# toastori/zig-flac

Hardware: AMD Instinct MI355X
Metric: MSamples/s encoded (whole node), 44.1kHz/16-bit stereo, blocksize 4096 (higher is better)
Workload: dtype int32

## Files before the change

### zig-flac_amd/csrc/fg_crc.hpp

```cpp
#pragma once
#include <stdint.h>

#ifndef FG_HD
#if defined(__HIPCC__)
#define FG_HD __host__ __device__ __forceinline__
#else
#define FG_HD inline
#endif
#endif

namespace fg {

FG_HD uint32_t q_fold(uint32_t t) {
    const uint32_t h = t >> 15;
    return (t & 0x7FFFu) ^ h ^ (h << 1);
}
FG_HD uint32_t q_word(uint32_t s, uint32_t W) { return q_fold(W ^ (s << 4) ^ (s << 2)); }
FG_HD uint32_t q_mul(uint32_t a, uint32_t e) {
    uint32_t r = 0;
#pragma unroll
    for (int i = 0; i < 15; i++) r ^= (e << i) & (uint32_t)(-(int32_t)((a >> i) & 1u));
    return q_fold(r);
}
FG_HD uint32_t crc_from_q(uint32_t qp) {
    const uint32_t A = qp & 0x7FFFu;
    return A ^ (((__builtin_popcount(A) ^ (qp >> 16)) & 1u) ? 0x8003u : 0u);
}
FG_HD uint32_t crc_lane_q(const uint32_t *img, int32_t va, uint32_t n, uint32_t e) {
    uint32_t s = 0, px = 0;
    for (uint32_t i = va < 0 ? (uint32_t)(-va) : 0u; i < n; i++) {
        const uint32_t w = img[va + (int32_t)i];
        s = q_word(s, w);
        px ^= w;
    }
    return q_mul(q_fold(s), e) | ((__builtin_popcount(px) & 1u) << 16);
}
FG_HD uint32_t crc_byte_v(uint32_t crc, uint32_t b) {
    const uint32_t t = ((crc >> 8) ^ b) & 255u;
    return ((crc << 8) ^ (t << 1) ^ (t << 2) ^ ((__builtin_popcount(t) & 1u) ? 0x8003u : 0u)) & 0xFFFFu;
}
FG_HD uint32_t crc_mulmod_v(uint32_t a, uint32_t b) {
    uint32_t t[16];
#pragma unroll
    for (int i = 0; i < 16; i++) t[i] = (b << i) & (uint32_t)(-(int32_t)((a >> i) & 1u));
#pragma unroll
    for (int w = 8; w >= 1; w >>= 1)
#pragma unroll
        for (int i = 0; i < w; i++) t[i] ^= t[i + w];
    return crc_from_q(q_fold(q_fold(t[0])) | ((__builtin_popcount(t[0]) & 1u) << 16));
}

}
```

### zig-flac_amd/csrc/fg_device.hpp

```cpp
#pragma once
#include <hip/hip_runtime.h>
#include <cstdlib>
#include <mutex>
#include <type_traits>

#include "fg_common.hpp"
#include "fg_crc.hpp"
#include "fg_layout.hpp"

namespace fg {

template <uint32_t V>
using ic = std::integral_constant<uint32_t, V>;
template <typename T>
struct tyt {
    using type = T;
};

__device__ __forceinline__ uint32_t lane_id() { return __lane_id(); }
__device__ __forceinline__ uint32_t opaque(uint32_t v) {
    asm volatile("" : "+v"(v));
    return v;
}

__device__ __forceinline__ uint32_t sad_u32(uint32_t a, uint32_t b, uint32_t acc) {
    uint32_t d;
    asm("v_sad_u32 %0, %1, %2, %3" : "=v"(d) : "v"(a), "v"(b), "v"(acc));
    return d;
}

__device__ __forceinline__ uint32_t add_chain(uint32_t a, uint32_t b) {
    uint32_t d;
    asm("v_add_u32 %0, %1, %2" : "=v"(d) : "v"(a), "v"(b));
    return d;
}

enum : int {
    DPP_XOR1 = 0xB1,
    DPP_XOR2 = 0x4E,
    DPP_SHR1 = 0x111,
    DPP_SHR2 = 0x112,
    DPP_SHR4 = 0x114,
    DPP_SHR8 = 0x118,
    DPP_WSHR1 = 0x138,
    DPP_MIRROR = 0x140,
    DPP_HMIRROR = 0x141,
    DPP_BCAST15 = 0x142,
    DPP_BCAST31 = 0x143,
};

template <int CTRL, int RM = 0xF, int BM = 0xF, bool BC = true>
__device__ __forceinline__ uint32_t dpp(uint32_t v) {
    return (uint32_t)__builtin_amdgcn_update_dpp(0, (int)v, CTRL, RM, BM, BC);
}
template <int CTRL>
__device__ __forceinline__ uint64_t dpp64(uint64_t v) {
    return (uint64_t)dpp<CTRL>((uint32_t)v) | ((uint64_t)dpp<CTRL>((uint32_t)(v >> 32)) << 32);
}
__device__ __forceinline__ uint32_t rdl(uint32_t v, int lane) {
    return (uint32_t)__builtin_amdgcn_readlane((int)v, lane);
}
__device__ __forceinline__ uint64_t rdl64(uint64_t v, int lane) {
    return (uint64_t)rdl((uint32_t)v, lane) | ((uint64_t)rdl((uint32_t)(v >> 32), lane) << 32);
}

template <typename T>
__device__ __forceinline__ T dppT(T v, int which);
#define FG_ROW_REDUCE(NAME, T, OP, DPPF)                       \
    __device__ __forceinline__ T NAME(T v) {                   \
        v = OP(v, DPPF<DPP_XOR1>(v));                          \
        v = OP(v, DPPF<DPP_XOR2>(v));                          \
        v = OP(v, DPPF<DPP_HMIRROR>(v));                       \
        v = OP(v, DPPF<DPP_MIRROR>(v));                        \
        return v;                                              \
    }
#define FG_ADD(a, b) ((a) + (b))
#define FG_OR(a, b) ((a) | (b))
#define FG_XOR(a, b) ((a) ^ (b))
#ifndef FG_MAX
#define FG_MAX(a, b) max((a), (b))
#endif
#ifndef FG_LKEEP24
#define FG_LKEEP24 1
#endif
FG_ROW_REDUCE(row_sum32, uint32_t, FG_ADD, dpp)
FG_ROW_REDUCE(row_sum64, uint64_t, FG_ADD, dpp64)
FG_ROW_REDUCE(row_or32, uint32_t, FG_OR, dpp)
FG_ROW_REDUCE(row_or64, uint64_t, FG_OR, dpp64)
FG_ROW_REDUCE(row_xor32, uint32_t, FG_XOR, dpp)
FG_ROW_REDUCE(row_max32, uint32_t, FG_MAX, dpp)

__device__ __forceinline__ uint32_t wave_sum32(uint32_t v) {
    v = row_sum32(v);
    return rdl(v, 0) + rdl(v, 16) + rdl(v, 32) + rdl(v, 48);
}
__device__ __forceinline__ uint64_t wave_sum64(uint64_t v) {
    v = row_sum64(v);
    return rdl64(v, 0) + rdl64(v, 16) + rdl64(v, 32) + rdl64(v, 48);
}
__device__ __forceinline__ uint32_t wave_or32(uint32_t v) {
    v = row_or32(v);
    return rdl(v, 0) | rdl(v, 16) | rdl(v, 32) | rdl(v, 48);
}
__device__ __forceinline__ uint64_t wave_or64(uint64_t v) {
    v = row_or64(v);
    return rdl64(v, 0) | rdl64(v, 16) | rdl64(v, 32) | rdl64(v, 48);
}
__device__ __forceinline__ uint32_t wave_max32(uint32_t v) {
    v = row_max32(v);
    return max(max(rdl(v, 0), rdl(v, 16)), max(rdl(v, 32), rdl(v, 48)));
}
__device__ __forceinline__ uint32_t wave_xor32(uint32_t v) {
    v = row_xor32(v);
    return rdl(v, 0) ^ rdl(v, 16) ^ rdl(v, 32) ^ rdl(v, 48);
}
__device__ __forceinline__ uint32_t wave_incl_scan32(uint32_t x) {
    x += dpp<DPP_SHR1>(x);
    x += dpp<DPP_SHR2>(x);
    x += dpp<DPP_SHR4>(x);
    x += dpp<DPP_SHR8>(x);
    x += dpp<DPP_BCAST15, 0xA, 0xF, false>(x);
    x += dpp<DPP_BCAST31, 0xC, 0xF, false>(x);
    return x;
}
__device__ __forceinline__ uint32_t shr1_32(uint32_t v) { return dpp<DPP_WSHR1>(v); }
__device__ __forceinline__ int32_t shr1(int32_t v) { return (int32_t)shr1_32((uint32_t)v); }
__device__ __forceinline__ int64_t shr1(int64_t v) { return (int64_t)dpp64<DPP_WSHR1>((uint64_t)v); }

__device__ __forceinline__ uint32_t bitlen32(uint32_t x) { return x ? 32u - (uint32_t)__builtin_clz(x) : 0u; }
__device__ __forceinline__ uint32_t bitlen64(uint64_t x) { return x ? 64u - (uint32_t)__builtin_clzll(x) : 0u; }
__device__ __forceinline__ uint32_t zigzag32(int32_t r) { return ((uint32_t)r << 1) ^ (uint32_t)(r >> 31); }

__device__ __forceinline__ uint32_t rice_choose(uint64_t S, uint32_t len, uint32_t width, uint32_t maxp,
                                                uint32_t *cost) {
    uint32_t p;
    if (S <= (uint64_t)((len + 1u) >> 1)) {
        p = 0;
    } else {
        const uint64_t two = 2ull * len;
        uint32_t m = 0;
        if (S > two) {
            m = bitlen64(S) - bitlen64(two);
            if ((S >> m) > two) m++;
        }
        p = m + 1u;
    }
    if (p > maxp - 1u) p = maxp - 1u;
    const uint64_t f = (p == 0) ? (uint64_t)len + (S << 1)
                                : (uint64_t)(1u + p) * len + ((S >> (p - 1u)) - (uint64_t)(len >> 1));
    const uint64_t esc = (width <= 31u) ? 5ull + (uint64_t)width * len : ~0ull;
    if (f < esc) {
        *cost = (uint32_t)f;
        return p;
    }
    *cost = (uint32_t)esc;
    return 0x80u | width;
}

__device__ __forceinline__ uint32_t rice_choose(uint32_t S, uint32_t len, uint32_t width, uint32_t maxp,
                                                uint32_t *cost) {
    uint32_t p;
    if (S <= ((len + 1u) >> 1)) {
        p = 0;
    } else {
        const uint32_t two = 2u * len;
        uint32_t m = 0;
        if (S > two) {
            m = bitlen32(S) - bitlen32(two);
            if ((S >> m) > two) m++;
        }
        p = m + 1u;
    }
    if (p > maxp - 1u) p = maxp - 1u;
    const uint32_t f = (p == 0) ? len + (S << 1) : (1u + p) * len + ((S >> (p - 1u)) - (len >> 1));
    const uint32_t esc = (width <= 31u) ? 5u + width * len : ~0u;
    if (f < esc) {
        *cost = f;
        return p;
    }
    *cost = esc;
    return 0x80u | width;
}


__device__ __forceinline__ void lds_or2(uint32_t addr, uint32_t hi, uint32_t lo) {
    asm volatile("ds_or_b32 %0, %1\n\tds_or_b32 %0, %2 offset:4" ::"v"(addr), "v"(hi), "v"(lo) : "memory");
}

__device__ __forceinline__ void store_frame16(const uint32_t *img, uint8_t *out, uint64_t D, uint32_t fbytes,
                                              uint32_t tid, uint32_t NT, uint32_t lo = 0) {
    const uint64_t E = D + fbytes;
    const uint32_t sa = (uint32_t)(D & 3u);
    const uint64_t qD = D >> 2;
    const uint64_t DL = D + lo;
    const uint32_t r = (uint32_t)(qD & 3u);
    for (uint64_t u = (DL >> 4) + tid; u < ((E + 15u) >> 4); u += NT) {
        const int32_t m0 = (int32_t)(4u * u - qD);
        const int32_t a1 = m0 + (int32_t)r;
        const uint4 q1 = *(const uint4 *)(img + a1);
        const uint4 q0 = a1 >= 4 ? *(const uint4 *)(img + a1 - 4) : make_uint4(0, 0, 0, 0);
        const uint32_t w8[8] = {q0.x, q0.y, q0.z, q0.w, q1.x, q1.y, q1.z, q1.w};
        uint32_t wv[5];
#pragma unroll
        for (int c = 0; c < 5; c++)
            wv[c] = r == 0 ? w8[3 + c] : r == 1 ? w8[2 + c] : r == 2 ? w8[1 + c] : w8[c];
        uint32_t v[4];
        uint32_t prev = m0 >= 1 ? wv[0] : 0u;
#pragma unroll
        for (int c = 0; c < 4; c++) {
            const uint32_t lo = m0 + c >= 0 ? wv[c + 1] : 0u;
            v[c] = __builtin_bswap32(sa ? __builtin_amdgcn_alignbyte(prev, lo, sa) : lo);
            prev = lo;
        }
        const uint64_t b0 = 16u * u;
        if (b0 >= DL && b0 + 16u <= E) {
            *(uint4 *)(out + b0) = make_uint4(v[0], v[1], v[2], v[3]);
        } else {
#pragma unroll
            for (int c = 0; c < 4; c++)
#pragma unroll
                for (uint32_t b = 0; b < 4; b++) {
                    const uint64_t bb = b0 + 4u * c + b;
                    if (bb >= DL && bb < E) out[bb] = (uint8_t)(v[c] >> (8 * b));
                }
        }
    }
}

__device__ __forceinline__ void put_bits(uint32_t *img, uint32_t pos, uint64_t v, uint32_t len) {
    if (len == 0) return;
    const uint32_t wi = pos >> 5, o = pos & 31u;
    const uint64_t t = v << (64u - o - len);
    atomicOr(&img[wi], (uint32_t)(t >> 32));
    if (o + len > 32u) atomicOr(&img[wi + 1], (uint32_t)t);
}

__device__ __forceinline__ void put_or2(uint32_t *img, uint32_t pos, uint64_t v, uint32_t len) {
    const uint32_t wi = pos >> 5, o = pos & 31u;
    const uint64_t t = len ? (v << (64u - o - len)) : 0ull;
    atomicOr(&img[wi], (uint32_t)(t >> 32));
    atomicOr(&img[wi + 1], (uint32_t)t);
}

struct AtomicWriter {
    uint32_t *img;
    uint32_t pos;
    __device__ __forceinline__ void init(uint32_t *im, uint32_t bitpos) {
        img = im;
        pos = bitpos;
    }
    __device__ __forceinline__ void put(uint64_t v, uint32_t len) {
        put_bits(img, pos, v, len);
        pos += len;
    }
    __device__ __forceinline__ void zeros(uint32_t q) { pos += q; }
    __device__ __forceinline__ void finish() {}
};

struct HdrWriter {
    uint64_t accu = 0;
    uint64_t w0 = 0;
    uint32_t remain = 64;
    uint32_t end = 0;
    __device__ void bits(uint32_t n, uint64_t v) {
        if (n == 0) return;
        if (n <= remain) {
            accu = (n == 64) ? 0 : (accu << n);
            accu |= v;
            remain -= n;
        } else {
            const uint32_t sh = n - remain;
            accu = (remain == 64) ? 0 : (accu << remain);
            accu |= v >> sh;
            w0 = accu;
            end++;
            accu = v;
            remain = 64 - sh;
        }
    }
};

__device__ __forceinline__ uint32_t crc8_byte(uint32_t c, uint32_t b) {
    c ^= b;
#pragma unroll
    for (int i = 0; i < 8; i++) c = (c & 0x80u) ? ((c << 1) ^ 0x07u) & 0xFFu : (c << 1) & 0xFFu;
    return c;
}

__device__ __noinline__ uint32_t write_frame_header(uint32_t *img, uint64_t frame_number, uint32_t bits,
                                                    uint32_t channel_code, uint32_t block_size,
                                                    uint32_t sample_rate) {
    HdrWriter h;
    h.bits(16, 0xFFF8);
    uint32_t unc_bs = 0;
    const uint32_t ctz = (uint32_t)__builtin_ctz(block_size);
    if ((block_size & (block_size - 1u)) == 0 && ctz <= 15 && ctz >= 8) {
        h.bits(4, ctz);
    } else if (block_size == 192) {
        h.bits(4, 1);
    } else if ((block_size >> ctz) == 144 && ctz <= 5 && ctz >= 2) {
        h.bits(4, ctz);
    } else if (block_size < 0x100) {
        h.bits(4, 6);
        unc_bs = 8;
    } else {
        h.bits(4, 7);
        unc_bs = 16;
    }
    uint32_t unc_sr = 0, rc;
    switch (sample_rate) {
        case 0: rc = 0; break;
        case 88200: rc = 1; break;
        case 176400: rc = 2; break;
        case 192000: rc = 3; break;
        case 8000: rc = 4; break;
        case 16000: rc = 5; break;
        case 22050: rc = 6; break;
        case 24000: rc = 7; break;
        case 32000: rc = 8; break;
        case 44100: rc = 9; break;
        case 48000: rc = 10; break;
        case 96000: rc = 11; break;
        default:
            if (sample_rate <= 255) { unc_sr = 4; rc = 12; }
            else if (sample_rate <= 65535) { unc_sr = 1; rc = 13; }
            else { unc_sr = 10; rc = 14; }
    }
    h.bits(4, rc);
    h.bits(4, channel_code);
    h.bits(4, bits == 8 ? 2u : bits == 16 ? 8u : bits == 24 ? 12u : 14u);
    if (frame_number <= 0x7F) {
        h.bits(8, frame_number);
    } else {
        uint64_t buf = 0, num = frame_number, fbm = 0x3F;
        uint32_t i = 0;
        while (num > fbm) {
            buf |= (0x80ull + (num & 0x3F)) << (8 * i);
            i++;
            num >>= 6;
            fbm >>= 1;
        }
        buf |= ((0xFEull << (6 - i)) | num) << (8 * i);
        const uint32_t nb = 8 * (i + 1);
        h.bits(nb, buf & (~0ull >> (64 - nb)));
    }
    if (unc_bs) h.bits(unc_bs, block_size - 1u);
    if (unc_sr == 4) h.bits(8, block_size);
    else if (unc_sr) h.bits(16, block_size / unc_sr);
    const uint32_t byte_end = 8u - h.remain / 8u;
    const uint64_t a_al = (h.remain == 64) ? h.accu : (h.accu << h.remain);
    const uint32_t nb = (h.end == 1 ? 8u : 0u) + byte_end;
    uint32_t c = 0;
    for (uint32_t q = 0; q < nb; q++) {
        const uint64_t src = (h.end == 1 && q < 8) ? h.w0 : a_al;
        const uint32_t qq = (h.end == 1 && q >= 8) ? q - 8 : q;
        const uint32_t byte = (uint32_t)(src >> (56 - 8 * qq)) & 255u;
        c = crc8_byte(c, byte);
        atomicOr(&img[q >> 2], byte << (24 - 8 * (q & 3)));
    }
    atomicOr(&img[nb >> 2], c << (24 - 8 * (nb & 3)));
    return nb + 1;
}

template <int CLS>
struct Cls {
    using S = typename std::conditional<CLS == 32, int64_t, int32_t>::type;
    using Sum = typename std::conditional<CLS == 16, uint32_t, uint64_t>::type;
};

template <int B>
__device__ __forceinline__ int32_t ld_sample(const uint8_t *p) {
    if constexpr (B == 1) return (int32_t)(*(const int8_t *)p);
    else if constexpr (B == 2) return (int32_t)(*(const int16_t *)p);
    else if constexpr (B == 3)
        return (int32_t)((uint32_t)p[0] | ((uint32_t)p[1] << 8)) | ((int32_t)(*(const int8_t *)(p + 2)) << 16);
    else return *(const int32_t *)p;
}

struct CandRes {
    uint32_t type, waste, bd, order, porder, method;
    int32_t lsh;
    uint64_t est;
    int64_t cval;
    __device__ __forceinline__ void make_uniform() {
        auto u32 = [](uint32_t v) { return (uint32_t)__builtin_amdgcn_readfirstlane((int)v); };
        auto u64 = [&](uint64_t v) { return (uint64_t)u32((uint32_t)v) | ((uint64_t)u32((uint32_t)(v >> 32)) << 32); };
        type = u32(type); waste = u32(waste); bd = u32(bd); order = u32(order); porder = u32(porder);
        method = u32(method); lsh = (int32_t)u32((uint32_t)lsh); est = u64(est); cval = (int64_t)u64((uint64_t)cval);
    }
};

#ifdef FG_STAMPS
#define STAMP(i)                                           \
    do {                                                   \
        const uint64_t t_ = __builtin_amdgcn_s_memtime(); \
        ph_[i] += t_ - tprev_;                             \
        tprev_ = t_;                                       \
    } while (0)
#else
#define STAMP(i) \
    do {         \
    } while (0)
#endif

#ifndef FG_DMA_ASM
#define FG_DMA_ASM 1
#endif
template <int SZ>
__device__ __forceinline__ void lds_dma(const void *g, void *lds) {
#if FG_DMA_ASM
    const uint32_t m = (uint32_t)__builtin_amdgcn_readfirstlane(
        (int)(uint32_t)(uintptr_t)(__attribute__((address_space(3))) void *)lds);
    uint32_t sv;
    if constexpr (SZ == 16)
        asm volatile("s_mov_b32 %0, m0\n\ts_mov_b32 m0, %1\n\ts_nop 0\n\tglobal_load_lds_dwordx4 %2, off\n\ts_mov_b32 m0, %0"
                     : "=&s"(sv) : "s"(m), "v"(g) : "memory");
    else
        asm volatile("s_mov_b32 %0, m0\n\ts_mov_b32 m0, %1\n\ts_nop 0\n\tglobal_load_lds_dword %2, off\n\ts_mov_b32 m0, %0"
                     : "=&s"(sv) : "s"(m), "v"(g) : "memory");
#else
    __builtin_amdgcn_global_load_lds((__attribute__((address_space(1))) void *)g,
                                     (__attribute__((address_space(3))) void *)lds, SZ, 0, 0);
#endif
}

__device__ __forceinline__ void stage_dma(const uint8_t *pcm, uint64_t off, uint32_t *stg, uint32_t cw, uint32_t cst,
                                          uint32_t wave, uint32_t NW, uint32_t l, bool ilv = false, uint32_t drh = 0,
                                          uint32_t half = 0) {
    const uint32_t *src = (const uint32_t *)(pcm + off);
    if (ilv) {
        for (uint32_t k = wave; k < 16u; k += NW)
            lds_dma<16>(src + (4u * k + (l & 3u)) * 64u + 4u * (l >> 2), stg + 272u * k);
        return;
    }
    if (drh) {
        const float inv = 1.0f / (float)drh;
        for (uint32_t ch = wave; ch < 64u; ch += NW) {
            for (uint32_t x0 = 0; x0 < cw; x0 += 64u) {
                const uint32_t x = x0 + l, r = (uint32_t)((float)x * inv), k = x - r * drh;
                if (x < cw)
                    lds_dma<4>(src + ch * 2u * cw + r * 2u * drh + half * drh + k, stg + ch * cst + x0);
            }
        }
        return;
    }
    for (uint32_t ch = wave; ch < 64u; ch += NW) {
        for (uint32_t x0 = 0; x0 < cw; x0 += 64u) {
            if (x0 + l < cw)
                lds_dma<4>(src + ch * cw + x0 + l, stg + ch * cst + x0);
        }
    }
}


__device__ __forceinline__ void bar_lds() { asm volatile("s_waitcnt lgkmcnt(0)\n\ts_barrier" ::: "memory"); }

__device__ __forceinline__ void reset_analysis_tickets(uint32_t *ctr, uint32_t tid) {
    if (blockIdx.x == 0 && tid < 16u && (tid < 2u || tid >= 8u)) ctr[tid] = 0u;
}

__device__ __forceinline__ uint32_t xcd_ticket(uint32_t *q, uint32_t n_frames) {
    uint32_t x;
    asm volatile("s_getreg_b32 %0, hwreg(HW_REG_XCC_ID)" : "=s"(x));
    x &= 7u;
    for (uint32_t i = 0; i < 8u; i++) {
        const uint32_t y = (x + i) & 7u;
        const uint32_t f0 = (uint32_t)(((uint64_t)n_frames * y) >> 3);
        const uint32_t f1 = (uint32_t)(((uint64_t)n_frames * (y + 1u)) >> 3);
        if (f1 == f0) continue;
        const uint32_t t = atomicAdd(&q[y], 1u);
        if (t < 2u * (f1 - f0)) return 2u * f0 + t;
    }
    return 0xFFFFFFFFu;
}

template <bool FULL>
__device__ __forceinline__ void stage_sync(const uint8_t *pcm, uint64_t off, uint32_t n, uint32_t CB, uint32_t *stg,
                                           uint32_t cw, uint32_t cst, uint32_t wave, uint32_t NW, uint32_t l,
                                           bool ilv = false) {
    const uint32_t in_bytes = n * CB;
    const uint32_t *src = (const uint32_t *)(pcm + off);
    const uint32_t nchunks = FULL ? 64u : (n + 63u) >> 6;
    for (uint32_t ch = wave; ch < nchunks; ch += NW) {
        for (uint32_t x = l; x < cw; x += 64) {
            const uint32_t wd = ch * cw + x;
            uint32_t v = 0;
            if (FULL || 4u * wd + 4u <= in_bytes) {
                v = src[wd];
            } else if (4u * wd < in_bytes) {
                const uint8_t *sb = (const uint8_t *)src + 4u * wd;
                for (uint32_t q = 0; 4u * wd + q < in_bytes; q++) v |= (uint32_t)sb[q] << (8 * q);
            }
            if (ilv) stg[272u * (ch >> 2) + 16u * (x >> 2) + 4u * (ch & 3u) + (x & 3u)] = v;
            else stg[ch * cst + x] = v;
        }
    }
}

template <int B, int CLS, bool FULL, int NC>
__device__ __forceinline__ void load_candidate(const uint32_t *stg, uint32_t cst, uint32_t l, uint32_t n, bool stereo,
                                               uint32_t cand, uint32_t C, typename Cls<CLS>::S (&s)[64]) {
    using ST = typename Cls<CLS>::S;
    const uint32_t *lw = stg + l * cst;
    const uint32_t kind = stereo ? cand : 0u;
    const uint32_t chan = stereo ? (cand == 1 ? 1u : 0u) : cand;
    auto fill = [&](auto getL, auto getR) {
#pragma unroll
        for (int g = 0; g < 4; g++) {
            if (kind <= 1) {
#pragma unroll
                for (int jj = 0; jj < 16; jj++) {
                    const int j = 16 * g + jj;
                    int64_t x = getL(j, chan);
                    if (!FULL && l * 64u + j >= n) x = 0;
                    s[j] = (ST)x;
                }
            } else if (kind == 2) {
#pragma unroll
                for (int jj = 0; jj < 16; jj++) {
                    const int j = 16 * g + jj;
                    int64_t x = (getL(j, 0u) + getR(j)) >> 1;
                    if (!FULL && l * 64u + j >= n) x = 0;
                    s[j] = (ST)x;
                }
            } else {
#pragma unroll
                for (int jj = 0; jj < 16; jj++) {
                    const int j = 16 * g + jj;
                    int64_t x = getL(j, 0u) - getR(j);
                    if (!FULL && l * 64u + j >= n) x = 0;
                    s[j] = (ST)x;
                }
            }
            __builtin_amdgcn_sched_barrier(0);
        }
    };
    if constexpr (NC == 2 && B == 4) {
        const uint2 *p2 = (const uint2 *)lw;
        fill([&](int j, uint32_t c) -> int64_t { return (int32_t)(c ? p2[j].y : p2[j].x); },
             [&](int j) -> int64_t { return (int32_t)p2[j].y; });
    } else if constexpr (NC == 2 && B == 2) {
        const uint4 *q4 = (const uint4 *)(stg + 272u * (l >> 2) + 4u * (l & 3u));
#pragma unroll
        for (int g = 0; g < 4; g++) {
            uint32_t raw[16];
#pragma unroll
            for (int t = 0; t < 4; t++) {
                const uint4 v = q4[4 * (4 * g + t)];
                raw[4 * t] = v.x; raw[4 * t + 1] = v.y; raw[4 * t + 2] = v.z; raw[4 * t + 3] = v.w;
            }
            auto put = [&](auto f) {
#pragma unroll
                for (int jj = 0; jj < 16; jj++) {
                    const int j = 16 * g + jj;
                    int32_t x = f((int32_t)(raw[jj] << 16) >> 16, (int32_t)raw[jj] >> 16);
                    if (!FULL && l * 64u + j >= n) x = 0;
                    s[j] = (ST)x;
                }
            };
            if (kind == 0 && chan == 0) put([](int32_t L, int32_t) { return L; });
            else if (kind <= 1) put([](int32_t, int32_t R) { return R; });
            else if (kind == 2) {
#pragma unroll
                for (int jj = 0; jj < 16; jj++) {
                    const int j = 16 * g + jj;
                    uint32_t sum;
                    asm("v_add_u32_sdwa %0, sext(%1), sext(%1) dst_sel:DWORD dst_unused:UNUSED_PAD src0_sel:WORD_0 src1_sel:WORD_1"
                        : "=v"(sum) : "v"(raw[jj]));
                    int32_t x = (int32_t)sum >> 1;
                    if (!FULL && l * 64u + j >= n) x = 0;
                    s[j] = (ST)x;
                }
            } else put([](int32_t L, int32_t R) { return L - R; });
            __builtin_amdgcn_sched_barrier(0);
        }
    } else if constexpr (B == 3) {
// ... 1965 lines not shown
```

### zig-flac_amd/csrc/fg_layout.hpp

```cpp
#pragma once
#include <stdint.h>

#include "fg_common.hpp"

namespace fg {

struct AnaLayout {
    uint32_t stage0;
    uint32_t stage1;
    uint32_t psum;
    uint32_t pmax;
    uint32_t par;
    uint32_t par_stride;
    uint32_t lpc;
    uint32_t rec;
    uint32_t misc;
    uint32_t lbits;
    uint32_t total;
};

struct PackLayout {
    uint32_t buf0;
    uint32_t buf1;
    uint32_t misc;
    uint32_t dsc;
    uint32_t total;
};

__host__ __device__ inline uint32_t fg_round16(uint32_t x) { return (x + 15u) & ~15u; }

__host__ __device__ inline bool stage_ilv(uint32_t C, uint32_t B) { return C == 2 && B == 2; }
__host__ __device__ inline uint32_t stage_pad(uint32_t C, uint32_t B) {
    return stage_ilv(C, B) ? 4u : ((C == 2 && B == 4) ? 2u : 1u);
}
__host__ __device__ inline uint32_t stage_bytes(uint32_t C, uint32_t B) {
    return 64u * (16u * C * B + stage_pad(C, B)) * 4u;
}

__host__ __device__ inline AnaLayout ana_layout(uint32_t C, uint32_t B, uint32_t nw, bool full, bool dbuf,
                                                bool lpc = false, uint32_t fused_img = 0) {
    AnaLayout L;
    uint32_t sb = fg_round16(stage_bytes(C, B));
    if (fused_img > sb) sb = fg_round16(fused_img);
    uint32_t end = sb;
    L.stage0 = L.stage1 = 0;
    if (full && dbuf) {
        L.stage1 = sb;
        end = 2u * sb;
    }
    L.psum = L.pmax = end;
    if (!full) {
        L.pmax = end + nw * 2048u;
        end += nw * 3072u;
    }
    L.par = end;
    L.par_stride = lpc ? 1024u : 512u;
    L.lpc = L.par + nw * L.par_stride;
    L.rec = L.lpc + (lpc ? nw * 4u * (uint32_t)kLpcTab : 0u);
    L.misc = L.rec + nw * 64u;
    L.lbits = L.misc + 256u;
    L.total = fg_round16(L.lbits + (fused_img ? 512u : 0u));
    return L;
}

__host__ __device__ inline PackLayout pack_layout(uint32_t C, uint32_t B, uint32_t image_bytes, bool dbuf) {
    PackLayout L;
    uint32_t r0 = stage_bytes(C, B);
    if (image_bytes > r0) r0 = image_bytes;
    r0 = fg_round16(r0);
    L.buf0 = 0;
    L.buf1 = dbuf ? r0 : 0u;
    L.misc = dbuf ? 2u * r0 : r0;
    L.dsc = L.misc + 256u;
    L.total = fg_round16(L.dsc);
    return L;
}

struct Ana1Layout {
    static constexpr uint32_t par = 0, rec = 2048, hdr = 2048 + 128, total = 2048 + 128 + 32;
};

struct P4Layout {
    uint32_t buf0, buf1, misc, dsc0, dsc1, total;
};
__host__ __device__ inline P4Layout pack4_layout(uint32_t image_bytes) {
    P4Layout L;
    uint32_t r0 = stage_bytes(2, 2);
    if (image_bytes > r0) r0 = image_bytes;
    r0 = fg_round16(r0);
    L.buf0 = 0;
    L.buf1 = r0;
    L.misc = 2u * r0;
    L.dsc0 = L.misc + 256u;
    L.dsc1 = L.dsc0 + 1280u;
    L.total = fg_round16(L.dsc1 + 1280u);
    return L;
}

__host__ __device__ inline uint32_t packw_cst(uint32_t C, uint32_t B, uint32_t wps) { return 16u * C * B + wps; }
__host__ __device__ inline uint32_t packw_dsc_hc(uint32_t nh) { return (18u + 11u * nh + 63u) / 64u; }
__host__ __device__ inline uint32_t packw_dsc_dw(uint32_t nh) { return 64u * (packw_dsc_hc(nh) + 2u * nh); }
__host__ __device__ inline PackLayout packw_layout(uint32_t C, uint32_t B, uint32_t wps, uint32_t image_bytes, bool dbuf,
                                                   uint32_t nh) {
    PackLayout L;
    uint32_t r0 = 64u * packw_cst(C, B, wps) * 4u;
    if (image_bytes > r0) r0 = image_bytes;
    r0 = fg_round16(r0);
    L.buf0 = 0;
    L.buf1 = dbuf ? r0 : 0u;
    L.misc = dbuf ? 2u * r0 : r0;
    L.dsc = L.misc + 256u;
    L.total = fg_round16(L.dsc + 2u * 4u * packw_dsc_dw(nh));
    return L;
}

__host__ __device__ inline uint32_t frame_bound_bytes(uint32_t n, uint32_t C, uint32_t bits, bool stereo) {
    uint64_t b = 16u * 8u;
    for (uint32_t c = 0; c < C; c++) {
        uint32_t bd = bits + ((stereo && c == 1) ? 1u : 0u);
        b += 14u + 4u * bd + (uint64_t)n * bd + n / 2u;
    }
    return (uint32_t)((b + 7u) / 8u + 1u + 2u + 16u);
}

}
```

### zig-flac_amd/csrc/fg_pack4.hpp

```cpp
#pragma once

#ifndef FG_PACK4_MINW
#define FG_PACK4_MINW 8
#endif


__device__ __forceinline__ void stage_dma_rot(const uint8_t *pcm, uint64_t off, uint32_t *stg, uint32_t wave,
                                              uint32_t NW, uint32_t l) {
    const uint32_t *src = (const uint32_t *)(pcm + off);
    for (uint32_t k = wave; k < 16u; k += NW) {
        const uint32_t j = 16u * k + (l >> 2);
        const uint32_t g = ((l & 3u) - (j >> 2)) & 3u;
        lds_dma<16>(src + 16u * j + 4u * g, stg + 256u * k);
    }
}

__device__ __forceinline__ uint32_t rot_off(uint32_t j, uint32_t g) { return 16u * j + 4u * ((g + (j >> 2)) & 3u); }

__device__ __forceinline__ void p4_dsc_dma(const EncodeArgs &a, uint32_t slot, uint32_t nxt_job, uint32_t *dsc,
                                           uint32_t wave, uint32_t l) {
    if (wave >= 5u) return;
    const uint8_t *fd = a.desc + (uint64_t)slot * a.desc_stride;
    const uint8_t *src;
    if (wave == 0) {
        if (l < 8u) src = fd + 4u * l;
        else if (l < 12u) src = fd + 32u + 4u * (l - 8u);
        else if (l < 16u) src = fd + 32u + sizeof(SubDesc) + 4u * (l - 12u);
        else if (l < 18u) src = (const uint8_t *)(a.offsets + slot) + 4u * (l - 16u);
        else if (l < 24u && nxt_job < a.n_jobs) src = (const uint8_t *)(a.jobs + nxt_job) + 4u * (l - 18u);
        else src = fd;
    } else if (wave <= 2u) {
        src = fd + 32u + (wave - 1u) * sizeof(SubDesc) + offsetof(SubDesc, lane_bits) + 4u * l;
    } else {
        src = fd + 32u + (wave - 3u) * sizeof(SubDesc) + offsetof(SubDesc, params) + 4u * l;
    }
    lds_dma<4>(src, dsc + 64u * wave);
}

template <int MAXT>
__global__ void __launch_bounds__(MAXT, FG_PACK4_MINW) k_pack4(EncodeArgs a) {
    if (a.enc_prio) __builtin_amdgcn_s_setprio(1);
    extern __shared__ __attribute__((aligned(16))) uint8_t smem[];

    const uint32_t tid = threadIdx.x, NT = blockDim.x, NW = NT >> 6;
    const uint32_t wave = (uint32_t)__builtin_amdgcn_readfirstlane((int)(tid >> 6)), l0 = lane_id();
    const uint32_t sfi = wave >> 2, qw = wave & 3u;
    const P4Layout LY = pack4_layout(a.image_bytes);
    uint32_t *misc = (uint32_t *)(smem + LY.misc);
    const bool stereo = a.stereo != 0;

    uint32_t *ctr = a.work_ctr + 2u;
    reset_analysis_tickets(a.work_ctr, tid);
    if (tid == 0) misc[21] = gridDim.x + atomicAdd(ctr, 1u);
    __syncthreads();
    uint32_t jidx = blockIdx.x, buf = 0;
    uint32_t nxt = (uint32_t)__builtin_amdgcn_readfirstlane((int)misc[21]);
    uint32_t tk = 0;
    if (tid == 0) tk = gridDim.x + atomicAdd(ctr, 1u);
    uint32_t slot = 0;
    if (jidx < a.n_jobs) {
        const FrameJob job = a.jobs[jidx];
        slot = job.slot;
        stage_dma_rot(a.pcm, job.pcm_off, (uint32_t *)(smem + LY.buf0), wave, NW, l0);
        p4_dsc_dma(a, job.slot, nxt, (uint32_t *)(smem + LY.dsc0), wave, l0);
    }
#ifdef FG_STAMPS
    uint64_t ph_[16] = {};
    uint64_t tprev_ = __builtin_amdgcn_s_memtime();
#endif
    const uint32_t i0 = 1024u * qw + 16u * l0;
    while (jidx < a.n_jobs) {
        const uint32_t l = opaque(l0);
        uint32_t *stg = (uint32_t *)(smem + (buf ? LY.buf1 : LY.buf0));
        uint32_t *img = stg;
        const uint32_t *dsc = (const uint32_t *)(smem + (buf ? LY.dsc1 : LY.dsc0));

        STAMP(7);
        if (tid == 0) misc[20] = tk;
        asm volatile("s_waitcnt vmcnt(0)" ::: "memory");
        STAMP(8);
        __syncthreads();
        STAMP(0);
        const uint32_t nn = (uint32_t)__builtin_amdgcn_readfirstlane((int)misc[20]);
        const uint32_t total_bits = (uint32_t)__builtin_amdgcn_readfirstlane((int)dsc[1]);
        const uint32_t fbytes = ((total_bits + 7u) >> 3) + 2u;
        const uint64_t D = ((uint64_t)(uint32_t)__builtin_amdgcn_readfirstlane((int)dsc[17]) << 32) |
                           (uint32_t)__builtin_amdgcn_readfirstlane((int)dsc[16]);
        const uint32_t Lb = (total_bits + 7u) >> 3;
        const uint32_t W4 = Lb >> 2;
        const uint32_t H = max((W4 + 2u * NT - 1u) / (2u * NT), 1u);
        const uint32_t hq = min(H, a.crc_hmax4) - 1u;
        const bool skip = fbytes + 16u > a.image_bytes || D + fbytes > a.out_cap;
        const uint32_t sdw0 = (uint32_t)__builtin_amdgcn_readfirstlane((int)dsc[8u + 4u * sfi]),
                       sdw1 = (uint32_t)__builtin_amdgcn_readfirstlane((int)dsc[9u + 4u * sfi]);
        const uint32_t type = sdw0 & 255u, w = (sdw0 >> 8) & 255u, bd = (sdw0 >> 16) & 255u, k = sdw0 >> 24,
                       o = sdw1 & 255u, method = (sdw1 >> 8) & 255u, cand = (sdw1 >> 16) & 255u;
        const uint32_t p = ((const uint8_t *)(dsc + 192u + 64u * sfi))[i0 >> (12u - o)];
        const uint32_t lb = dsc[64u + 64u * sfi + l];
        uint32_t sub_start = 8u * (uint32_t)__builtin_amdgcn_readfirstlane((int)dsc[0]);
        if (sfi) sub_start += (uint32_t)__builtin_amdgcn_readfirstlane((int)dsc[10]);
        const uint32_t hdrw = dsc[4u + (l & 3u)];
        const uint64_t jn_off = ((uint64_t)(uint32_t)__builtin_amdgcn_readfirstlane((int)dsc[19]) << 32) |
                                (uint32_t)__builtin_amdgcn_readfirstlane((int)dsc[18]);
        const uint32_t jn_slot = (uint32_t)__builtin_amdgcn_readfirstlane((int)dsc[23]);
        const uint32_t crc_pw = a.crc_pow4[hq * NT + tid];
        if (nxt < a.n_jobs) {
            stage_dma_rot(a.pcm, jn_off, (uint32_t *)(smem + (buf ? LY.buf0 : LY.buf1)), wave, NW, l);
            p4_dsc_dma(a, jn_slot, nn, (uint32_t *)(smem + (buf ? LY.dsc0 : LY.dsc1)), wave, l);
        }
        if (skip) {
            if (tid == 0) {
                atomicOr(a.err, fbytes + 16u > a.image_bytes ? 1u : 2u);
                tk = gridDim.x + atomicAdd(ctr, 1u);
            }
            __syncthreads();
            jidx = nxt; nxt = nn; slot = jn_slot; buf ^= 1u;
            continue;
        }
        const uint32_t j = 64u * qw + l;
        uint32_t raw[20];
        {
            const uint4 hv = j ? *(const uint4 *)(stg + rot_off(j - 1u, 3u)) : make_uint4(0, 0, 0, 0);
            raw[0] = hv.x; raw[1] = hv.y; raw[2] = hv.z; raw[3] = hv.w;
#pragma unroll
            for (int g = 0; g < 4; g++) {
                const uint4 v = *(const uint4 *)(stg + rot_off(j, (uint32_t)g));
                raw[4 + 4 * g] = v.x; raw[5 + 4 * g] = v.y; raw[6 + 4 * g] = v.z; raw[7 + 4 * g] = v.w;
            }
        }
        STAMP(9);
        const uint32_t kind = stereo ? cand : (cand ? 1u : 0u);
        int32_t x[20];
        auto unpack = [&](auto KD) {
            constexpr uint32_t KND = decltype(KD)::value;
#pragma unroll
            for (int i = 0; i < 20; i++) {
                const int32_t L = (int32_t)(raw[i] << 16) >> 16, R = (int32_t)raw[i] >> 16;
                x[i] = KND == 0 ? L : KND == 1 ? R : KND == 2 ? (L + R) >> 1 : L - R;
            }
        };
        if (kind == 0) unpack(ic<0>{});
        else if (kind == 1) unpack(ic<1>{});
        else if (kind == 2) unpack(ic<2>{});
        else unpack(ic<3>{});
        const uint32_t lbs = wave_incl_scan32(lb);
        const uint32_t qbase = qw ? rdl(lbs, (int)(16u * qw - 1u)) : 0u;
        STAMP(10);
        bar_lds();
        STAMP(1);
        const uint32_t Wz = (fbytes + 3u) / 4u + 2u;
        for (uint32_t i = tid; i < Wz; i += NT) img[i] = 0;
        STAMP(2);

        const uint32_t bps = bd - w;
        if (type != 0 && w != 0) {
#pragma unroll
            for (int i = 0; i < 20; i++) x[i] >>= w;
        }
        const bool first = (qw == 0) && (l == 0);
        const uint32_t param_len = 4u + method;
        const bool esc = (p & 0x80u) != 0;
        const uint32_t wb = p & 0x7Fu, pr = esc ? 0u : p;
        uint32_t r[16];
        auto resid = [&](auto KO) {
            constexpr uint32_t K = decltype(KO)::value;
#pragma unroll
            for (int i = 0; i < 16; i++) {
                const uint32_t u0 = (uint32_t)x[4 + i], u1 = (uint32_t)x[3 + i], u2 = (uint32_t)x[2 + i],
                               u3 = (uint32_t)x[1 + i], u4 = (uint32_t)x[i];
                if constexpr (K == 0) r[i] = u0;
                else if constexpr (K == 1) r[i] = u0 - u1;
                else if constexpr (K == 2) r[i] = (u0 + u2) - 2u * u1;
                else if constexpr (K == 3) r[i] = (u0 - u3) + 3u * (u2 - u1);
                else r[i] = (u0 + u4) - 4u * (u1 + u3) + 6u * u2;
            }
        };
        if (type != 2 || k == 0) resid(ic<0>{});
        else if (k == 1) resid(ic<1>{});
        else if (k == 2) resid(ic<2>{});
        else if (k == 3) resid(ic<3>{});
        else resid(ic<4>{});
        const uint32_t cl = esc ? wb : pr + 1u;
        const uint32_t cmask = esc ? ((1u << wb) - 1u) : ((1u << pr) - 1u);
        const uint32_t cbit = esc ? 0u : (1u << pr);
        const uint32_t qmask = esc ? 0u : ~0u;
        const uint32_t nwarm = (first && type == 2) ? k : 0u;
        auto warm_at = [&](int i) -> bool { return i < 4 && (uint32_t)i < nwarm; };
        uint32_t len = 0;
        if (first) {
            if (type == 0) len = 8u + bd;
            else if (type == 1) len = 8u + w;
            else len = 8u + w + k * bps + 6u + param_len + (esc ? 5u : 0u);
        } else if (type == 2 && (i0 & ((4096u >> o) - 1u)) == 0) {
            len = param_len + (esc ? 5u : 0u);
        }
        if (type == 1) {
            len += 16u * bps;
        } else if (type == 2) {
            uint32_t qs = 0;
#pragma unroll
            for (int i = 0; i < 16; i++) {
                const uint32_t qz = zigzag32((int32_t)r[i]) >> pr;
                qs = add_chain(qs, warm_at(i) ? 0u : qz);
            }
            len += (qs & qmask) + (16u - nwarm) * cl;
        }
        const uint32_t lane_off = wave_incl_scan32(len) - len;
        bar_lds();
        STAMP(3);
        if (tid < 4 && hdrw) atomicOr(&img[tid], hdrw);

        {
            uint32_t pos = sub_start + qbase + lane_off;
            const uint64_t mask = ~0ull >> (64 - (bps ? bps : 1u));
            if (first) {
                AtomicWriter bw;
                bw.init(img, pos);
                if (type == 0) {
                    bw.put(0, 8);
                    const SubDesc *sd = (const SubDesc *)(a.desc + (uint64_t)slot * a.desc_stride + sizeof(FrameDesc)) + sfi;
                    bw.put(((uint64_t)sd->cval << w) & (~0ull >> (64 - bd)), bd);
                } else {
                    const uint32_t tc = (type == 1) ? 1u : (8u | k);
                    bw.put((tc << 1) | (w ? 1u : 0u), 8);
                    if (w) bw.put(1, w);
                    if (type == 2) {
#pragma unroll
                        for (int i = 0; i < 4; i++)
                            if ((uint32_t)i < k) bw.put((uint64_t)(int64_t)x[4 + i] & mask, bps);
                        bw.put((method << 4) | o, 6);
                        if (esc) {
                            bw.put(0x0Fu | (method << 4), 4u + method);
                            bw.put(wb, 5);
                        } else {
                            bw.put(p, 4u + method);
                        }
                    }
                }
                pos = bw.pos;
            } else if (type == 2 && (i0 & ((4096u >> o) - 1u)) == 0) {
                const uint32_t esc_code = (0x0Fu | (method << 4)) << 5;
                const uint32_t hl = param_len + (esc ? 5u : 0u);
                put_or2(img, pos, esc ? (esc_code | wb) : p, hl);
                pos += hl;
            }
            if (type == 1) {
#pragma unroll
                for (int i = 0; i < 16; i++) {
                    put_or2(img, pos, (uint64_t)(int64_t)(int32_t)r[i] & mask, bps);
                    pos += bps;
                }
            } else if (type == 2) {
                const uint32_t img_lds = (uint32_t)(uintptr_t)(__attribute__((address_space(3))) uint32_t *)img;
                uint32_t pa = 8u * img_lds + pos;
                const uint32_t ncl = 64u - cl;
                auto emit = [&](auto ESC) {
                    constexpr bool E = decltype(ESC)::value != 0;
#pragma unroll
                    for (int i = 0; i < 16; i++) {
                        const bool warm = warm_at(i);
                        const uint32_t zz = zigzag32((int32_t)r[i]);
                        const uint32_t src = E ? (esc ? r[i] : zz) : zz;
                        uint32_t v = (src & cmask) | cbit;
                        uint32_t q = E ? ((zz >> pr) & qmask) : (zz >> pr);
                        uint32_t sh = ncl, adv = cl;
                        if (i < 4) {
                            v = warm ? 0u : v;
                            q = warm ? 0u : q;
                            sh = warm ? 64u : sh;
                            adv = warm ? 0u : adv;
                        }
                        pa += q;
                        const uint64_t t = (uint64_t)v << ((sh - (pa & 31u)) & 63u);
                        lds_or2((pa >> 3) & ~3u, (uint32_t)(t >> 32), (uint32_t)t);
                        pa += adv;
                    }
                };
                if (__any(esc)) emit(ic<1>{});
                else emit(ic<0>{});
            }
        }
        bar_lds();
        STAMP(4);

        {
            const int32_t Z = (int32_t)(NT * 2u * H) - (int32_t)W4;
            const int32_t va = (int32_t)(tid * 2u * H) - Z;
            uint32_t contrib = crc_lane_q(img, va, 2u * H, crc_pw);
            contrib = wave_xor32(contrib);
            if (l == 0) misc[wave] = contrib;
        }
        bar_lds();
        if (tid == 0) {
            uint32_t qp = 0;
            for (uint32_t i = 0; i < NW; i++) qp ^= misc[i];
            uint32_t crc = crc_from_q(qp);
            for (uint32_t b = W4 * 4u; b < Lb; b++)
                crc = crc_byte_v(crc, (img[b >> 2] >> (24 - 8 * (b & 3))) & 255u);
            put_bits(img, Lb * 8u, crc, 16);
        }
        bar_lds();
        STAMP(5);

        store_frame16(img, a.out, D, fbytes, tid, NT);
        STAMP(6);
        if (tid == 0) tk = gridDim.x + atomicAdd(ctr, 1u);
        jidx = nxt; nxt = nn; slot = jn_slot; buf ^= 1u;
    }
#ifdef FG_STAMPS
    if (l0 == 0 && a.stamps)
        for (int i = 0; i < 11; i++) atomicAdd(&a.stamps[16 + i], (unsigned long long)ph_[i]);
#endif
}
```

Baseline: 152,200.

## Retune pack4 kernel codegen: compile-time wave count, scalar pinning, vectorized CRC and stores

Makes the thread count a compile-time constant and pins uniform values (wave, grid size, layout, stereo flag, kernarg pointer) into scalar registers, mainly to cut vector-register pressure inside the frame loop. The CRC lane fold gets vectorized 2- and 4-word paths, and waves that hold no CRC data skip the fold. The output store uses 32-bit offsets and word-granular partial writes instead of per-byte stores. The zero fill now uses uint4 stores, zigzag values are computed once and reused, and the LDS DMA is driven by raw LDS addresses in an unrolled loop. In exchange the code is harder to read and the escape path must now undo the zigzag.

New measurement: 153,600, median of 6. Within noise of the previous version (+0.9%).

```diff
diff --git a/zig-flac_amd/csrc/fg_crc.hpp b/zig-flac_amd/csrc/fg_crc.hpp
--- a/zig-flac_amd/csrc/fg_crc.hpp
+++ b/zig-flac_amd/csrc/fg_crc.hpp
@@ -19,19 +19,64 @@
 FG_HD uint32_t q_mul(uint32_t a, uint32_t e) {
     uint32_t r = 0;
 #pragma unroll
-    for (int i = 0; i < 15; i++) r ^= (e << i) & (uint32_t)(-(int32_t)((a >> i) & 1u));
+    for (int i = 0; i < 15; i++) {
+        r ^= e & (uint32_t)((int32_t)(a << (31 - i)) >> 31);
+        e <<= 1;
+    }
     return q_fold(r);
 }
 FG_HD uint32_t crc_from_q(uint32_t qp) {
     const uint32_t A = qp & 0x7FFFu;
     return A ^ (((__builtin_popcount(A) ^ (qp >> 16)) & 1u) ? 0x8003u : 0u);
 }
+template <int N>
+FG_HD void crc_load_block(uint32_t *dst, const uint32_t *src) {
+    __builtin_memcpy(dst, __builtin_assume_aligned(src, 4 * N), 4 * N);
+}
+template <int N>
+FG_HD uint32_t crc_fold_words(const uint32_t *w, uint32_t *px) {
+    uint32_t s = 0, x = 0;
+#pragma unroll
+    for (int c = 0; c < N; c++) {
+        s = q_word(s, w[c]);
+        x ^= w[c];
+    }
+    *px = x;
+    return s;
+}
+FG_HD uint32_t crc_uniform(uint32_t v) {
+#if defined(__HIP_DEVICE_COMPILE__)
+    return (uint32_t)__builtin_amdgcn_readfirstlane((int)v);
+#else
+    return v;
+#endif
+}
 FG_HD uint32_t crc_lane_q(const uint32_t *img, int32_t va, uint32_t n, uint32_t e) {
     uint32_t s = 0, px = 0;
-    for (uint32_t i = va < 0 ? (uint32_t)(-va) : 0u; i < n; i++) {
-        const uint32_t w = img[va + (int32_t)i];
-        s = q_word(s, w);
-        px ^= w;
+    if (n == 4u) {
+        const int32_t b = va & ~3;
+        const uint32_t r = crc_uniform((uint32_t)va & 3u);
+        uint32_t w8[8] = {0, 0, 0, 0, 0, 0, 0, 0};
+        if (b >= 0) crc_load_block<4>(w8, img + b);
+        if (r != 0 && b + 4 >= 0) crc_load_block<4>(w8 + 4, img + b + 4);
+        if (r == 0) s = crc_fold_words<4>(w8, &px);
+        else if (r == 1) s = crc_fold_words<4>(w8 + 1, &px);
+        else if (r == 2) s = crc_fold_words<4>(w8 + 2, &px);
+        else s = crc_fold_words<4>(w8 + 3, &px);
+    } else if (n == 2u) {
+        const int32_t b = va & ~1;
+        const uint32_t r = crc_uniform((uint32_t)va & 1u);
+        uint32_t w4[4] = {0, 0, 0, 0};
+        if (b >= 0) crc_load_block<2>(w4, img + b);
+        if (r != 0 && b + 2 >= 0) crc_load_block<2>(w4 + 2, img + b + 2);
+        if (r == 0) s = crc_fold_words<2>(w4, &px);
+        else s = crc_fold_words<2>(w4 + 1, &px);
+    } else {
+        for (uint32_t i = va < 0 ? (uint32_t)(-va) : 0u; i < n; i++) {
+            const uint32_t w = img[va + (int32_t)i];
+            s = q_word(s, w);
+            px ^= w;
+        }
     }
     return q_mul(q_fold(s), e) | ((__builtin_popcount(px) & 1u) << 16);
 }
diff --git a/zig-flac_amd/csrc/fg_device.hpp b/zig-flac_amd/csrc/fg_device.hpp
--- a/zig-flac_amd/csrc/fg_device.hpp
+++ b/zig-flac_amd/csrc/fg_device.hpp
@@ -20,6 +20,10 @@
 __device__ __forceinline__ uint32_t lane_id() { return __lane_id(); }
 __device__ __forceinline__ uint32_t opaque(uint32_t v) {
     asm volatile("" : "+v"(v));
+    return v;
+}
+__device__ __forceinline__ uint32_t opaque_s(uint32_t v) {
+    asm volatile("" : "+s"(v));
     return v;
 }
 
@@ -189,14 +193,14 @@
 
 __device__ __forceinline__ void store_frame16(const uint32_t *img, uint8_t *out, uint64_t D, uint32_t fbytes,
                                               uint32_t tid, uint32_t NT, uint32_t lo = 0) {
-    const uint64_t E = D + fbytes;
-    const uint32_t sa = (uint32_t)(D & 3u);
-    const uint64_t qD = D >> 2;
-    const uint64_t DL = D + lo;
-    const uint32_t r = (uint32_t)(qD & 3u);
-    for (uint64_t u = (DL >> 4) + tid; u < ((E + 15u) >> 4); u += NT) {
-        const int32_t m0 = (int32_t)(4u * u - qD);
-        const int32_t a1 = m0 + (int32_t)r;
+    const uint32_t d = (uint32_t)D & 15u;
+    uint8_t *base = out + (D - d);
+    const uint32_t beg = d + lo, end = d + fbytes;
+    const uint32_t sa = d & 3u;
+    const uint32_t r = d >> 2;
+    for (uint32_t u = (beg >> 4) + tid; u < ((end + 15u) >> 4); u += NT) {
+        const int32_t a1 = (int32_t)(4u * u);
+        const int32_t m0 = a1 - (int32_t)r;
         const uint4 q1 = *(const uint4 *)(img + a1);
         const uint4 q0 = a1 >= 4 ? *(const uint4 *)(img + a1 - 4) : make_uint4(0, 0, 0, 0);
         const uint32_t w8[8] = {q0.x, q0.y, q0.z, q0.w, q1.x, q1.y, q1.z, q1.w};
@@ -212,17 +216,26 @@
             v[c] = __builtin_bswap32(sa ? __builtin_amdgcn_alignbyte(prev, lo, sa) : lo);
             prev = lo;
         }
-        const uint64_t b0 = 16u * u;
-        if (b0 >= DL && b0 + 16u <= E) {
-            *(uint4 *)(out + b0) = make_uint4(v[0], v[1], v[2], v[3]);
+        const uint32_t b0 = 16u * u;
+        if (b0 >= beg && b0 + 16u <= end) {
+            *(uint4 *)(base + b0) = make_uint4(v[0], v[1], v[2], v[3]);
         } else {
 #pragma unroll
-            for (int c = 0; c < 4; c++)
-#pragma unroll
-                for (uint32_t b = 0; b < 4; b++) {
-                    const uint64_t bb = b0 + 4u * c + b;
-                    if (bb >= DL && bb < E) out[bb] = (uint8_t)(v[c] >> (8 * b));
-                }
+            for (uint32_t c = 0; c < 4; c++)
+                if (b0 + 4u * c >= beg && b0 + 4u * c + 4u <= end) *(uint32_t *)(base + b0 + 4u * c) = v[c];
+            const uint32_t hb = beg & 3u, hc = (beg >> 2) & 3u, tb = end & 3u, tc = (end >> 2) & 3u;
+            if (hb && u == (beg >> 4)) {
+                const uint32_t hv = hc == 0 ? v[0] : hc == 1 ? v[1] : hc == 2 ? v[2] : v[3];
+#pragma unroll
+                for (uint32_t b = 1; b < 4; b++)
+                    if (b >= hb && (beg & ~3u) + b < end) base[(beg & ~3u) + b] = (uint8_t)(hv >> (8 * b));
+            }
+            if (tb && u == (end >> 4) && !(hb && (beg >> 2) == (end >> 2))) {
+                const uint32_t tv = tc == 0 ? v[0] : tc == 1 ? v[1] : tc == 2 ? v[2] : v[3];
+#pragma unroll
+                for (uint32_t b = 0; b < 3; b++)
+                    if (b < tb) base[(end & ~3u) + b] = (uint8_t)(tv >> (8 * b));
+            }
         }
     }
 }
@@ -422,6 +435,17 @@
     __builtin_amdgcn_global_load_lds((__attribute__((address_space(1))) void *)g,
                                      (__attribute__((address_space(3))) void *)lds, SZ, 0, 0);
 #endif
+}
+template <int SZ>
+__device__ __forceinline__ void lds_dma_at(const void *g, uint32_t lds_addr) {
+    const uint32_t m = (uint32_t)__builtin_amdgcn_readfirstlane((int)lds_addr);
+    uint32_t sv;
+    if constexpr (SZ == 16)
+        asm volatile("s_mov_b32 %0, m0\n\ts_mov_b32 m0, %1\n\ts_nop 0\n\tglobal_load_lds_dwordx4 %2, off\n\ts_mov_b32 m0, %0"
+                     : "=&s"(sv) : "s"(m), "v"(g) : "memory");
+    else
+        asm volatile("s_mov_b32 %0, m0\n\ts_mov_b32 m0, %1\n\ts_nop 0\n\tglobal_load_lds_dword %2, off\n\ts_mov_b32 m0, %0"
+                     : "=&s"(sv) : "s"(m), "v"(g) : "memory");
 }
 
 __device__ __forceinline__ void stage_dma(const uint8_t *pcm, uint64_t off, uint32_t *stg, uint32_t cw, uint32_t cst,
diff --git a/zig-flac_amd/csrc/fg_layout.hpp b/zig-flac_amd/csrc/fg_layout.hpp
--- a/zig-flac_amd/csrc/fg_layout.hpp
+++ b/zig-flac_amd/csrc/fg_layout.hpp
@@ -83,11 +83,8 @@
 struct P4Layout {
     uint32_t buf0, buf1, misc, dsc0, dsc1, total;
 };
-__host__ __device__ inline P4Layout pack4_layout(uint32_t image_bytes) {
+__host__ __device__ inline P4Layout pack4_layout_r0(uint32_t r0) {
     P4Layout L;
-    uint32_t r0 = stage_bytes(2, 2);
-    if (image_bytes > r0) r0 = image_bytes;
-    r0 = fg_round16(r0);
     L.buf0 = 0;
     L.buf1 = r0;
     L.misc = 2u * r0;
@@ -95,6 +92,11 @@
     L.dsc1 = L.dsc0 + 1280u;
     L.total = fg_round16(L.dsc1 + 1280u);
     return L;
+}
+__host__ __device__ inline P4Layout pack4_layout(uint32_t image_bytes) {
+    uint32_t r0 = stage_bytes(2, 2);
+    if (image_bytes > r0) r0 = image_bytes;
+    return pack4_layout_r0(fg_round16(r0));
 }
 
 __host__ __device__ inline uint32_t packw_cst(uint32_t C, uint32_t B, uint32_t wps) { return 16u * C * B + wps; }
diff --git a/zig-flac_amd/csrc/fg_pack4.hpp b/zig-flac_amd/csrc/fg_pack4.hpp
--- a/zig-flac_amd/csrc/fg_pack4.hpp
+++ b/zig-flac_amd/csrc/fg_pack4.hpp
@@ -5,19 +5,21 @@
 #endif
 
 
-__device__ __forceinline__ void stage_dma_rot(const uint8_t *pcm, uint64_t off, uint32_t *stg, uint32_t wave,
-                                              uint32_t NW, uint32_t l) {
+template <uint32_t NW>
+__device__ __forceinline__ void stage_dma_rot(const uint8_t *pcm, uint64_t off, uint32_t stg, uint32_t wave, uint32_t l) {
     const uint32_t *src = (const uint32_t *)(pcm + off);
-    for (uint32_t k = wave; k < 16u; k += NW) {
+#pragma unroll
+    for (uint32_t i = 0; i < 16u / NW; i++) {
+        const uint32_t k = wave + i * NW;
         const uint32_t j = 16u * k + (l >> 2);
         const uint32_t g = ((l & 3u) - (j >> 2)) & 3u;
-        lds_dma<16>(src + 16u * j + 4u * g, stg + 256u * k);
+        lds_dma_at<16>(src + 16u * j + 4u * g, stg + 1024u * k);
     }
 }
 
 __device__ __forceinline__ uint32_t rot_off(uint32_t j, uint32_t g) { return 16u * j + 4u * ((g + (j >> 2)) & 3u); }
 
-__device__ __forceinline__ void p4_dsc_dma(const EncodeArgs &a, uint32_t slot, uint32_t nxt_job, uint32_t *dsc,
+__device__ __forceinline__ void p4_dsc_dma(const EncodeArgs &a, uint32_t slot, uint32_t nxt_job, uint32_t dsc,
                                            uint32_t wave, uint32_t l) {
     if (wave >= 5u) return;
     const uint8_t *fd = a.desc + (uint64_t)slot * a.desc_stride;
@@ -34,49 +36,65 @@
     } else {
         src = fd + 32u + (wave - 3u) * sizeof(SubDesc) + offsetof(SubDesc, params) + 4u * l;
     }
-    lds_dma<4>(src, dsc + 64u * wave);
+    lds_dma_at<4>(src, dsc + 256u * wave);
 }
 
+__device__ __forceinline__ const __attribute__((address_space(4))) EncodeArgs *p4_kernargs() {
+    uint64_t v = (uint64_t)(uintptr_t)__builtin_amdgcn_kernarg_segment_ptr();
+    asm volatile("" : "+s"(v));
+    return (const __attribute__((address_space(4))) EncodeArgs *)v;
+}
+
 template <int MAXT>
-__global__ void __launch_bounds__(MAXT, FG_PACK4_MINW) k_pack4(EncodeArgs a) {
+__global__ void __attribute__((amdgpu_flat_work_group_size(MAXT, MAXT), amdgpu_waves_per_eu(FG_PACK4_MINW, FG_PACK4_MINW)))
+k_pack4(EncodeArgs a) {
     if (a.enc_prio) __builtin_amdgcn_s_setprio(1);
     extern __shared__ __attribute__((aligned(16))) uint8_t smem[];
 
-    const uint32_t tid = threadIdx.x, NT = blockDim.x, NW = NT >> 6;
-    const uint32_t wave = (uint32_t)__builtin_amdgcn_readfirstlane((int)(tid >> 6)), l0 = lane_id();
-    const uint32_t sfi = wave >> 2, qw = wave & 3u;
-    const P4Layout LY = pack4_layout(a.image_bytes);
-    uint32_t *misc = (uint32_t *)(smem + LY.misc);
-    const bool stereo = a.stereo != 0;
+    constexpr uint32_t NT = MAXT, NW = MAXT / 64;
+    static_assert(16u % NW == 0 && NW >= 5u, "DMA pieces per wave; the descriptor DMA uses waves 0..4");
+    const uint32_t tid0 = threadIdx.x;
+    const uint32_t wave0 = (uint32_t)__builtin_amdgcn_readfirstlane((int)(tid0 >> 6)), l0 = lane_id();
+    const uint32_t smem_lds = (uint32_t)(uintptr_t)(__attribute__((address_space(3))) uint8_t *)smem;
+    const P4Layout LY0 = pack4_layout(a.image_bytes);
+    uint32_t *misc0 = (uint32_t *)(smem + LY0.misc);
 
     uint32_t *ctr = a.work_ctr + 2u;
-    reset_analysis_tickets(a.work_ctr, tid);
-    if (tid == 0) misc[21] = gridDim.x + atomicAdd(ctr, 1u);
+    const uint32_t grid = opaque_s(gridDim.x);
+    reset_analysis_tickets(a.work_ctr, tid0);
+    if (tid0 == 0) misc0[21] = grid + atomicAdd(ctr, 1u);
     __syncthreads();
     uint32_t jidx = blockIdx.x, buf = 0;
-    uint32_t nxt = (uint32_t)__builtin_amdgcn_readfirstlane((int)misc[21]);
+    uint32_t nxt = (uint32_t)__builtin_amdgcn_readfirstlane((int)misc0[21]);
     uint32_t tk = 0;
-    if (tid == 0) tk = gridDim.x + atomicAdd(ctr, 1u);
+    if (tid0 == 0) tk = grid + atomicAdd(ctr, 1u);
     uint32_t slot = 0;
     if (jidx < a.n_jobs) {
         const FrameJob job = a.jobs[jidx];
         slot = job.slot;
-        stage_dma_rot(a.pcm, job.pcm_off, (uint32_t *)(smem + LY.buf0), wave, NW, l0);
-        p4_dsc_dma(a, job.slot, nxt, (uint32_t *)(smem + LY.dsc0), wave, l0);
+        stage_dma_rot<NW>(a.pcm, job.pcm_off, smem_lds + LY0.buf0, wave0, l0);
+        p4_dsc_dma(a, job.slot, nxt, smem_lds + LY0.dsc0, wave0, l0);
     }
 #ifdef FG_STAMPS
     uint64_t ph_[16] = {};
     uint64_t tprev_ = __builtin_amdgcn_s_memtime();
 #endif
-    const uint32_t i0 = 1024u * qw + 16u * l0;
     while (jidx < a.n_jobs) {
         const uint32_t l = opaque(l0);
+        const uint32_t wave = opaque_s(wave0), tid = 64u * wave + l;
+        const uint32_t sfi = wave >> 2, qw = wave & 3u;
+        const uint32_t i0 = 1024u * qw + 16u * l;
+        const P4Layout LY = pack4_layout_r0(opaque_s(LY0.buf1));
+        uint32_t *misc = (uint32_t *)(smem + LY.misc);
+        const auto *ka = p4_kernargs();
         uint32_t *stg = (uint32_t *)(smem + (buf ? LY.buf1 : LY.buf0));
         uint32_t *img = stg;
         const uint32_t *dsc = (const uint32_t *)(smem + (buf ? LY.dsc1 : LY.dsc0));
 
         STAMP(7);
         if (tid == 0) misc[20] = tk;
+        const uint32_t image_bytes = ka->image_bytes;
+        const uint64_t out_cap = ka->out_cap;
         asm volatile("s_waitcnt vmcnt(0)" ::: "memory");
         STAMP(8);
         __syncthreads();
@@ -90,7 +108,7 @@
         const uint32_t W4 = Lb >> 2;
         const uint32_t H = max((W4 + 2u * NT - 1u) / (2u * NT), 1u);
         const uint32_t hq = min(H, a.crc_hmax4) - 1u;
-        const bool skip = fbytes + 16u > a.image_bytes || D + fbytes > a.out_cap;
+        const bool skip = fbytes + 16u > image_bytes || D + fbytes > out_cap;
         const uint32_t sdw0 = (uint32_t)__builtin_amdgcn_readfirstlane((int)dsc[8u + 4u * sfi]),
                        sdw1 = (uint32_t)__builtin_amdgcn_readfirstlane((int)dsc[9u + 4u * sfi]);
         const uint32_t type = sdw0 & 255u, w = (sdw0 >> 8) & 255u, bd = (sdw0 >> 16) & 255u, k = sdw0 >> 24,
@@ -103,15 +121,15 @@
         const uint64_t jn_off = ((uint64_t)(uint32_t)__builtin_amdgcn_readfirstlane((int)dsc[19]) << 32) |
                                 (uint32_t)__builtin_amdgcn_readfirstlane((int)dsc[18]);
         const uint32_t jn_slot = (uint32_t)__builtin_amdgcn_readfirstlane((int)dsc[23]);
-        const uint32_t crc_pw = a.crc_pow4[hq * NT + tid];
+        const uint32_t crc_pw = opaque(a.crc_pow4[hq * NT + tid]);
         if (nxt < a.n_jobs) {
-            stage_dma_rot(a.pcm, jn_off, (uint32_t *)(smem + (buf ? LY.buf0 : LY.buf1)), wave, NW, l);
-            p4_dsc_dma(a, jn_slot, nn, (uint32_t *)(smem + (buf ? LY.dsc0 : LY.dsc1)), wave, l);
+            stage_dma_rot<NW>(a.pcm, jn_off, smem_lds + (buf ? LY.buf0 : LY.buf1), wave, l);
+            p4_dsc_dma(a, jn_slot, nn, smem_lds + (buf ? LY.dsc0 : LY.dsc1), wave, l);
         }
         if (skip) {
             if (tid == 0) {
-                atomicOr(a.err, fbytes + 16u > a.image_bytes ? 1u : 2u);
-                tk = gridDim.x + atomicAdd(ctr, 1u);
+                atomicOr(ka->err, fbytes + 16u > image_bytes ? 1u : 2u);
+                tk = grid + atomicAdd(ctr, 1u);
             }
             __syncthreads();
             jidx = nxt; nxt = nn; slot = jn_slot; buf ^= 1u;
@@ -129,7 +147,7 @@
             }
         }
         STAMP(9);
-        const uint32_t kind = stereo ? cand : (cand ? 1u : 0u);
+        const uint32_t kind = opaque_s(a.stereo) ? cand : (cand ? 1u : 0u);
         int32_t x[20];
         auto unpack = [&](auto KD) {
             constexpr uint32_t KND = decltype(KD)::value;
@@ -149,7 +167,7 @@
         bar_lds();
         STAMP(1);
         const uint32_t Wz = (fbytes + 3u) / 4u + 2u;
-        for (uint32_t i = tid; i < Wz; i += NT) img[i] = 0;
+        for (uint32_t i = tid; 4u * i < Wz; i += NT) ((uint4 *)img)[i] = make_uint4(0, 0, 0, 0);
         STAMP(2);
 
         const uint32_t bps = bd - w;
@@ -200,8 +218,8 @@
             uint32_t qs = 0;
 #pragma unroll
             for (int i = 0; i < 16; i++) {
-                const uint32_t qz = zigzag32((int32_t)r[i]) >> pr;
-                qs = add_chain(qs, warm_at(i) ? 0u : qz);
+                r[i] = zigzag32((int32_t)r[i]);
+                qs = add_chain(qs, warm_at(i) ? 0u : r[i] >> pr);
             }
             len += (qs & qmask) + (16u - nwarm) * cl;
         }
@@ -218,7 +236,7 @@
                 bw.init(img, pos);
                 if (type == 0) {
                     bw.put(0, 8);
-                    const SubDesc *sd = (const SubDesc *)(a.desc + (uint64_t)slot * a.desc_stride + sizeof(FrameDesc)) + sfi;
+                    const SubDesc *sd = (const SubDesc *)(ka->desc + (uint64_t)slot * ka->desc_stride + sizeof(FrameDesc)) + sfi;
                     bw.put(((uint64_t)sd->cval << w) & (~0ull >> (64 - bd)), bd);
                 } else {
                     const uint32_t tc = (type == 1) ? 1u : (8u | k);
@@ -259,8 +277,8 @@
 #pragma unroll
                     for (int i = 0; i < 16; i++) {
                         const bool warm = warm_at(i);
-                        const uint32_t zz = zigzag32((int32_t)r[i]);
-                        const uint32_t src = E ? (esc ? r[i] : zz) : zz;
+                        const uint32_t zz = r[i];
+                        const uint32_t src = E ? (esc ? (zz >> 1) ^ (0u - (zz & 1u)) : zz) : zz;
                         uint32_t v = (src & cmask) | cbit;
                         uint32_t q = E ? ((zz >> pr) & qmask) : (zz >> pr);
                         uint32_t sh = ncl, adv = cl;
@@ -285,14 +303,17 @@
 
         {
             const int32_t Z = (int32_t)(NT * 2u * H) - (int32_t)W4;
-            const int32_t va = (int32_t)(tid * 2u * H) - Z;
-            uint32_t contrib = crc_lane_q(img, va, 2u * H, crc_pw);
-            contrib = wave_xor32(contrib);
+            uint32_t contrib = 0;
+            if ((int32_t)((wave + 1u) * 128u * H) > Z) {
+                contrib = wave_xor32(crc_lane_q(img, (int32_t)(tid * 2u * H) - Z, 2u * H, crc_pw));
+            }
             if (l == 0) misc[wave] = contrib;
         }
+        uint8_t *const out = ka->out;
         bar_lds();
         if (tid == 0) {
             uint32_t qp = 0;
+#pragma unroll
             for (uint32_t i = 0; i < NW; i++) qp ^= misc[i];
             uint32_t crc = crc_from_q(qp);
             for (uint32_t b = W4 * 4u; b < Lb; b++)
@@ -302,9 +323,9 @@
         bar_lds();
         STAMP(5);
 
-        store_frame16(img, a.out, D, fbytes, tid, NT);
+        store_frame16(img, out, D, fbytes, tid, NT);
         STAMP(6);
-        if (tid == 0) tk = gridDim.x + atomicAdd(ctr, 1u);
+        if (tid == 0) tk = grid + atomicAdd(ctr, 1u);
         jidx = nxt; nxt = nn; slot = jn_slot; buf ^= 1u;
     }
 #ifdef FG_STAMPS
```
